# cambrian-mllm/cambrian

Hardware: NVIDIA H100
Metric: train_samples_per_sec (higher is better)
Workload: dtype bf16

## Files before the change

cambrian_b200/csrc/gemm.cu:

```cuda
#include "common.cuh"
#include <algorithm>
#include <cstring>
#include <cudaTypedefs.h>
#include <mutex>

namespace cb {

constexpr int BM = 128;
constexpr int BK = 64;
constexpr int GEMM_THREADS = 288;
constexpr int GROUP_M = 16;

struct GemmEpilogue {
  void* C;
  long long ldc, bsc;
  const bf16* bias;
  const bf16* colscale;
  const bf16* residual;
  long long ldr, bsr;
  float alpha;
  int out_fp32;
  int accumulate;
  int pair_ok;
  int tma_store;
};
constexpr int ACT_SWIGLU_PAIR = 5;

constexpr int STG_BYTES = 64 * 64 * 2;
constexpr int STAGING_BYTES = 2 * 2 * STG_BYTES;

template <int BN>
struct GemmCfg {
  static constexpr int A_BYTES = BM * BK * 2;
  static constexpr int B_BYTES = BN * BK * 2;
  static constexpr int STAGE_BYTES = A_BYTES + B_BYTES;
  static constexpr int STAGES = (BN == 256) ? 4 : (BN == 128 ? 6 : 8);
  static constexpr int SMEM_BYTES = STAGES * STAGE_BYTES + STAGING_BYTES + 1024  + 256 ;
  static_assert(SMEM_BYTES <= 232448, "exceeds the 227 KB of shared memory a CTA may use");
};

template <int ACT>
__device__ __forceinline__ float apply_act(float v) {
  if constexpr (ACT == 1) return gelu_erf(v);
  else if constexpr (ACT == 2) return gelu_tanh_fast(v);
  else if constexpr (ACT == 3) return quick_gelu(v);
  else if constexpr (ACT == 4) return silu(v);
  else return v;
}

__device__ __forceinline__ void tile_to_mn(int r, int m_blocks, int n_blocks, int& mb, int& nb) {
  const int tpg = GROUP_M * n_blocks;
  const int g = r / tpg;
  const int first = g * GROUP_M;
  const int gs = min(GROUP_M, m_blocks - first);
  const int w = r - g * tpg;
  mb = first + w % gs;
  nb = w / gs;
}

template <int BN, int ACT>
__device__ __forceinline__ void fuse_row(const GemmEpilogue& ep, long long c_off, long long r_off, int col0, int N,
                                         float* acc, int h) {
  constexpr int J = BN / 8;
#pragma unroll
  for (int j = 0; j < J; ++j) {
    acc[4 * j + 2 * h] *= ep.alpha;
    acc[4 * j + 2 * h + 1] *= ep.alpha;
  }
  if (ep.bias) {
#pragma unroll
    for (int j = 0; j < J; ++j) {
      const int col = col0 + 8 * j;
      if (col < N) {
        const float2 t = __bfloat1622float2(*reinterpret_cast<const __nv_bfloat162*>(ep.bias + col));
        acc[4 * j + 2 * h] += t.x;
        acc[4 * j + 2 * h + 1] += t.y;
      }
    }
  }
  if constexpr (ACT != 0) {
#pragma unroll
    for (int j = 0; j < J; ++j) {
      acc[4 * j + 2 * h] = apply_act<ACT>(acc[4 * j + 2 * h]);
      acc[4 * j + 2 * h + 1] = apply_act<ACT>(acc[4 * j + 2 * h + 1]);
    }
  }
  if (ep.colscale) {
#pragma unroll
    for (int j = 0; j < J; ++j) {
      const int col = col0 + 8 * j;
      if (col < N) {
        const float2 t = __bfloat1622float2(*reinterpret_cast<const __nv_bfloat162*>(ep.colscale + col));
        acc[4 * j + 2 * h] *= t.x;
        acc[4 * j + 2 * h + 1] *= t.y;
      }
    }
  }
  if (ep.residual) {
#pragma unroll
    for (int j = 0; j < J; ++j) {
      const int col = col0 + 8 * j;
      if (col < N) {
        const float2 t = __bfloat1622float2(*reinterpret_cast<const __nv_bfloat162*>(ep.residual + r_off + col));
        acc[4 * j + 2 * h] += t.x;
        acc[4 * j + 2 * h + 1] += t.y;
      }
    }
  }
  if (ep.accumulate && ep.out_fp32) {
    const float* cr = reinterpret_cast<const float*>(ep.C) + c_off;
#pragma unroll
    for (int j = 0; j < J; ++j) {
      const int col = col0 + 8 * j;
      if (col < N) {
        const float2 o = *reinterpret_cast<const float2*>(cr + col);
        acc[4 * j + 2 * h] += o.x;
        acc[4 * j + 2 * h + 1] += o.y;
      }
    }
  } else if (ep.accumulate) {
    const bf16* cr = reinterpret_cast<const bf16*>(ep.C) + c_off;
#pragma unroll
    for (int j = 0; j < J; ++j) {
      const int col = col0 + 8 * j;
      if (col < N) {
        const float2 o = __bfloat1622float2(*reinterpret_cast<const __nv_bfloat162*>(cr + col));
        acc[4 * j + 2 * h] += o.x;
        acc[4 * j + 2 * h + 1] += o.y;
      }
    }
  }
}

template <int BN>
__device__ __forceinline__ void store_row(const GemmEpilogue& ep, long long c_off, int col0, int N, const float* acc,
                                          int h) {
#pragma unroll
  for (int j = 0; j < BN / 8; ++j) {
    const int col = col0 + 8 * j;
    if (col >= N) continue;
    const float x = acc[4 * j + 2 * h], y = acc[4 * j + 2 * h + 1];
    if (ep.out_fp32) *reinterpret_cast<float2*>(reinterpret_cast<float*>(ep.C) + c_off + col) = make_float2(x, y);
    else *reinterpret_cast<__nv_bfloat162*>(reinterpret_cast<bf16*>(ep.C) + c_off + col) = __floats2bfloat162_rn(x, y);
  }
}

template <int ACT>
__device__ __forceinline__ void epilogue_elems(const GemmEpilogue& ep, long long c_off, long long r_off, int col, int N,
                                               float v0, float v1) {
  v0 *= ep.alpha;
  v1 *= ep.alpha;
#pragma unroll
  for (int e = 0; e < 2; ++e) {
    const int c = col + e;
    if (c >= N) break;
    float v = e ? v1 : v0;
    if (ep.bias) v += __bfloat162float(ep.bias[c]);
    v = apply_act<ACT>(v);
    if (ep.colscale) v *= __bfloat162float(ep.colscale[c]);
    if (ep.residual) v += __bfloat162float(ep.residual[r_off + c]);
    if (ep.out_fp32) {
      float* cp = reinterpret_cast<float*>(ep.C) + c_off + c;
      *cp = ep.accumulate ? *cp + v : v;
    } else {
      bf16* cp = reinterpret_cast<bf16*>(ep.C) + c_off + c;
      *cp = __float2bfloat16(ep.accumulate ? __bfloat162float(*cp) + v : v);
    }
  }
}

template <int BN, bool A_MN, bool B_MN, int ACT>
__global__ void __launch_bounds__(GEMM_THREADS, 1)
gemm_bf16_wgmma(const __grid_constant__ CUtensorMap tmA, const __grid_constant__ CUtensorMap tmB,
                const __grid_constant__ CUtensorMap tmC, const __grid_constant__ CUtensorMap tmAux, int M, int N, int K,
                int tiles, GemmEpilogue ep) {
  using Cfg = GemmCfg<BN>;
  constexpr int STAGES = Cfg::STAGES;
  constexpr bool SWIGLU = ACT == ACT_SWIGLU_PAIR;
  extern __shared__ uint8_t smem_raw[];
  const uint32_t smem_base = (smem_u32(smem_raw) + 1023u) & ~1023u;
  const uint32_t stg_base = smem_base + STAGES * Cfg::STAGE_BYTES;
  const uint32_t bar_base = stg_base + STAGING_BYTES;
  auto full_bar = [&](int s) { return bar_base + 8u * s; };
  auto empty_bar = [&](int s) { return bar_base + 8u * (STAGES + s); };

  const int warp = threadIdx.x >> 5;
  const int lane = threadIdx.x & 31;
  const int m_blocks = (M + BM - 1) / BM;
  const int n_blocks = SWIGLU ? (N / 2) / (BN / 2) : (N + BN - 1) / BN;
  const int tiles_per_batch = m_blocks * n_blocks;
  const int num_kb = (K + BK - 1) / BK;

  if (warp == 8 && lane == 0) {
    tma_prefetch_desc(&tmA);
    tma_prefetch_desc(&tmB);
    for (int s = 0; s < STAGES; ++s) {
      mbar_init(full_bar(s), 1);
      mbar_init(empty_bar(s), 2);
    }
    mbar_fence_init();
  }
  __syncthreads();

  if (warp == 8) {
    if (lane == 0) {
      int stage = 0;
      uint32_t phase = 0;
      for (int r = blockIdx.x; r < tiles; r += gridDim.x) {
        const int b = r / tiles_per_batch;
        int mb, nb;
        tile_to_mn(r - b * tiles_per_batch, m_blocks, n_blocks, mb, nb);
        const int m0 = mb * BM;
        for (int kb = 0; kb < num_kb; ++kb) {
          mbar_wait(empty_bar(stage), phase ^ 1u);
          const uint32_t sa = smem_base + stage * Cfg::STAGE_BYTES;
          const uint32_t sb = sa + Cfg::A_BYTES;
          mbar_arrive_expect_tx(full_bar(stage), Cfg::STAGE_BYTES);
          const int k0 = kb * BK;
          if (!A_MN) {
            tma_load_3d(sa, &tmA, full_bar(stage), k0, m0, b);
          } else {
#pragma unroll
            for (int i = 0; i < BM / 64; ++i)
              tma_load_3d(sa + i * (64 * BK * 2), &tmA, full_bar(stage), m0 + 64 * i, k0, b);
          }
          if (SWIGLU) {
            tma_load_3d(sb, &tmB, full_bar(stage), k0, nb * (BN / 2), 0);
            tma_load_3d(sb + (BN / 2) * BK * 2, &tmB, full_bar(stage), k0, N / 2 + nb * (BN / 2), 0);
          } else if (!B_MN) {
            tma_load_3d(sb, &tmB, full_bar(stage), k0, nb * BN, b);
          } else {
#pragma unroll
            for (int i = 0; i < BN / 64; ++i)
              tma_load_3d(sb + i * (64 * BK * 2), &tmB, full_bar(stage), nb * BN + 64 * i, k0, b);
          }
          if (++stage == STAGES) {
            stage = 0;
            phase ^= 1u;
          }
        }
      }
    }
    return;
  }

  const int wg = warp >> 2;
  const bool wg_leader = (threadIdx.x & 127) == 0;
  const int srow = (warp & 3) * 16 + (lane >> 2);
  const int cq = 2 * (lane & 3);
  const uint32_t stg = stg_base + wg * (2 * STG_BYTES);
  uint32_t q = 0;
  if (wg_leader && ep.tma_store) {
    tma_prefetch_desc(&tmC);
    if (SWIGLU) tma_prefetch_desc(&tmAux);
  }

  auto store_subtile = [&](const CUtensorMap* map, int x, int x_end, int y, int z, auto pair) {
    const uint32_t buf = stg + (q & 1u) * STG_BYTES;
#pragma unroll
    for (int h = 0; h < 2; ++h) {
      const int row = srow + 8 * h;
#pragma unroll
      for (int j = 0; j < 8; ++j) {
        const __nv_bfloat162 v = pair(j, h);
        st_shared_b32(buf + row * 128 + ((j ^ (row & 7)) << 4) + 2 * cq, *reinterpret_cast<const uint32_t*>(&v));
      }
    }
    fence_proxy_async_smem();
    if (wg_leader) bulk_wait_read<0>();
    named_bar_sync(1 + wg, 128);
    if (wg_leader && x < x_end && y < M) {
      tma_store_3d(map, buf, x, y, z);
      bulk_commit();
    }
    ++q;
  };

  float acc[BN / 2];
  int stage = 0;
  uint32_t phase = 0;
  for (int r = blockIdx.x; r < tiles; r += gridDim.x) {
    const int b = r / tiles_per_batch;
    int mb, nb;
    tile_to_mn(r - b * tiles_per_batch, m_blocks, n_blocks, mb, nb);
    const int m0 = mb * BM;
#pragma unroll
    for (int i = 0; i < BN / 2; ++i) acc[i] = 0.f;
    int prev_stage = -1;
    for (int kb = 0; kb < num_kb; ++kb) {
      mbar_wait(full_bar(stage), phase);
      const uint32_t sa = smem_base + stage * Cfg::STAGE_BYTES + wg * (64 * 128);
      const uint32_t sb = smem_base + stage * Cfg::STAGE_BYTES + Cfg::A_BYTES;
      reg_fence(acc);
      wgmma_fence();
#pragma unroll
      for (int k = 0; k < BK / 16; ++k) {
        const uint64_t adesc = A_MN ? make_smem_desc_sw128(sa + k * 2048, 64 * BK * 2, 1024)
                                    : make_smem_desc_sw128(sa + k * 32, 0, 1024);
        const uint64_t bdesc = B_MN ? make_smem_desc_sw128(sb + k * 2048, 64 * BK * 2, 1024)
                                    : make_smem_desc_sw128(sb + k * 32, 0, 1024);
        WgmmaSS<BN, A_MN ? 1 : 0, B_MN ? 1 : 0>::mma(acc, adesc, bdesc, 1u);
      }
      wgmma_commit();
      wgmma_wait<1>();
      reg_fence(acc);
      if (prev_stage >= 0 && wg_leader) mbar_arrive(empty_bar(prev_stage));
      prev_stage = stage;
      if (++stage == STAGES) {
        stage = 0;
        phase ^= 1u;
      }
    }
    wgmma_wait<0>();
    reg_fence(acc);
    if (wg_leader) mbar_arrive(empty_bar(prev_stage));

    const int y0 = m0 + wg * 64;
    if constexpr (SWIGLU) {
      constexpr int JH = BN / 16;
      const int F = N >> 1;
      const int f0 = nb * (BN / 2);
#pragma unroll
      for (int s = 0; s < BN / 128; ++s)
        store_subtile(&tmC, f0 + 64 * s, N, y0, 0, [&](int j, int h) {
          return __floats2bfloat162_rn(acc[4 * (8 * s + j) + 2 * h], acc[4 * (8 * s + j) + 2 * h + 1]);
        });
#pragma unroll
      for (int s = 0; s < BN / 128; ++s)
        store_subtile(&tmC, F + f0 + 64 * s, N, y0, 0, [&](int j, int h) {
          return __floats2bfloat162_rn(acc[4 * (JH + 8 * s + j) + 2 * h], acc[4 * (JH + 8 * s + j) + 2 * h + 1]);
        });
#pragma unroll
      for (int s = 0; s < BN / 128; ++s)
        store_subtile(&tmAux, f0 + 64 * s, F, y0, 0, [&](int j, int h) {
          const float2 g = __bfloat1622float2(
              __floats2bfloat162_rn(acc[4 * (8 * s + j) + 2 * h], acc[4 * (8 * s + j) + 2 * h + 1]));
          const float2 u = __bfloat1622float2(
              __floats2bfloat162_rn(acc[4 * (JH + 8 * s + j) + 2 * h], acc[4 * (JH + 8 * s + j) + 2 * h + 1]));
          return __floats2bfloat162_rn(silu(g.x) * u.x, silu(g.y) * u.y);
        });
    } else {
      const int n0 = nb * BN;
#pragma unroll
      for (int h = 0; h < 2; ++h) {
        const int row = y0 + srow + 8 * h;
        if (row >= M) continue;
        const long long c_off = static_cast<long long>(b) * ep.bsc + static_cast<long long>(row) * ep.ldc;
        const long long r_off = static_cast<long long>(b) * ep.bsr + static_cast<long long>(row) * ep.ldr;
        if (ep.pair_ok) {
          fuse_row<BN, ACT>(ep, c_off, r_off, n0 + cq, N, acc, h);
          if (!ep.tma_store) store_row<BN>(ep, c_off, n0 + cq, N, acc, h);
          continue;
        }
#pragma unroll
        for (int j = 0; j < BN / 8; ++j) {
          if (n0 + 8 * j >= N) break;
          epilogue_elems<ACT>(ep, c_off, r_off, n0 + 8 * j + cq, N, acc[4 * j + 2 * h], acc[4 * j + 2 * h + 1]);
        }
      }
      if (ep.tma_store) {
#pragma unroll
        for (int s = 0; s < BN / 64; ++s)
          store_subtile(&tmC, n0 + 64 * s, N, y0, b, [&](int j, int h) {
            return __floats2bfloat162_rn(acc[4 * (8 * s + j) + 2 * h], acc[4 * (8 * s + j) + 2 * h + 1]);
          });
      }
    }
  }
  if (wg_leader) bulk_wait<0>();
}

static PFN_cuTensorMapEncodeTiled_v12000 get_encode_fn() {
  static PFN_cuTensorMapEncodeTiled_v12000 fn = nullptr;
  static std::once_flag once;
  std::call_once(once, [] {
    void* p = nullptr;
    cudaDriverEntryPointQueryResult q;
    if (cudaGetDriverEntryPoint("cuTensorMapEncodeTiled", &p, cudaEnableDefault, &q) == cudaSuccess &&
        q == cudaDriverEntryPointSuccess)
      fn = reinterpret_cast<PFN_cuTensorMapEncodeTiled_v12000>(p);
  });
  return fn;
}

int make_tmap_bf16_3d(CUtensorMap* out, const void* base, uint64_t inner, uint64_t rows, uint64_t batch,
                      uint64_t ld_elems, uint64_t batch_stride_elems, uint32_t box_rows) {
  auto fn = get_encode_fn();
  if (!fn) return set_error(CB_ERR_CUDA, "cuTensorMapEncodeTiled entry point not available");
  if ((reinterpret_cast<uintptr_t>(base) & 15u) != 0)
    return set_error(CB_ERR_INVALID, "TMA operand base must be 16-byte aligned");
  if ((ld_elems % 8) != 0 || (batch > 1 && (batch_stride_elems % 8) != 0))
    return set_error(CB_ERR_INVALID, "TMA operand strides must be multiples of 8 elements (ld=%llu)",
                     (unsigned long long)ld_elems);
  cuuint64_t dims[3] = {inner, rows, batch};
  cuuint64_t bs = (batch > 1) ? batch_stride_elems * 2 : ld_elems * 2 * (rows ? rows : 1);
  cuuint64_t strides[2] = {ld_elems * 2, bs};
  cuuint32_t box[3] = {64, box_rows, 1};
  cuuint32_t estr[3] = {1, 1, 1};
  CUresult r = fn(out, CU_TENSOR_MAP_DATA_TYPE_BFLOAT16, 3, const_cast<void*>(base), dims, strides, box,
                  estr, CU_TENSOR_MAP_INTERLEAVE_NONE, CU_TENSOR_MAP_SWIZZLE_128B,
                  CU_TENSOR_MAP_L2_PROMOTION_L2_256B, CU_TENSOR_MAP_FLOAT_OOB_FILL_NONE);
  if (r == CUDA_ERROR_INVALID_CONTEXT) {
    cudaFree(0);
    r = fn(out, CU_TENSOR_MAP_DATA_TYPE_BFLOAT16, 3, const_cast<void*>(base), dims, strides, box, estr,
           CU_TENSOR_MAP_INTERLEAVE_NONE, CU_TENSOR_MAP_SWIZZLE_128B, CU_TENSOR_MAP_L2_PROMOTION_L2_256B,
           CU_TENSOR_MAP_FLOAT_OOB_FILL_NONE);
  }
  if (r != CUDA_SUCCESS) return set_error(CB_ERR_CUDA, "cuTensorMapEncodeTiled failed (%d)", (int)r);
  return CB_OK;
}

struct GemmMaps {
  CUtensorMap a, b, c, aux;
};

template <int BN, bool A_MN, bool B_MN, int ACT>
static int launch_gemm(const GemmMaps& tm, int M, int N, int K, int batch, const GemmEpilogue& ep,
                       cudaStream_t stream) {
  using Cfg = GemmCfg<BN>;
  auto kern = gemm_bf16_wgmma<BN, A_MN, B_MN, ACT>;
  static bool attr_set = false;
  if (!attr_set) {
    cudaError_t e = cudaFuncSetAttribute(kern, cudaFuncAttributeMaxDynamicSharedMemorySize, Cfg::SMEM_BYTES);
    if (e != cudaSuccess) return set_error(CB_ERR_CUDA, "gemm smem attr: %s", cudaGetErrorString(e));
    attr_set = true;
  }
  const int n_blocks = (ACT == ACT_SWIGLU_PAIR) ? (N / 2) / (BN / 2) : (N + BN - 1) / BN;
  const long long tiles = (long long)((M + BM - 1) / BM) * n_blocks * batch;
  CB_CHECK_ARG(tiles < (1LL << 31), "gemm: %lld tiles exceed the grid", tiles);
  const unsigned grid = (unsigned)std::min<long long>(tiles, device_sm_count());
  kern<<<grid, GEMM_THREADS, Cfg::SMEM_BYTES, stream>>>(tm.a, tm.b, tm.c, tm.aux, M, N, K, (int)tiles, ep);
  CB_CUDA_LAUNCH_CHECK("gemm_bf16_wgmma");
  return CB_OK;
}

template <int BN>
static int dispatch_major(int a_mn, int b_mn, int act, const GemmMaps& tm, int M, int N, int K, int batch,
                          const GemmEpilogue& ep, cudaStream_t stream) {
  if (!a_mn && !b_mn) {
    switch (act) {
      case 1: return launch_gemm<BN, false, false, 1>(tm, M, N, K, batch, ep, stream);
      case 2: return launch_gemm<BN, false, false, 2>(tm, M, N, K, batch, ep, stream);
      case 3: return launch_gemm<BN, false, false, 3>(tm, M, N, K, batch, ep, stream);
      case 4: return launch_gemm<BN, false, false, 4>(tm, M, N, K, batch, ep, stream);
      default: return launch_gemm<BN, false, false, 0>(tm, M, N, K, batch, ep, stream);
    }
  }
  if (!a_mn && b_mn) return launch_gemm<BN, false, true, 0>(tm, M, N, K, batch, ep, stream);
  if (a_mn && !b_mn) return launch_gemm<BN, true, false, 0>(tm, M, N, K, batch, ep, stream);
  return launch_gemm<BN, true, true, 0>(tm, M, N, K, batch, ep, stream);
}

int gemm_bf16(const void* A, const void* B, void* C, int M, int N, int K, int batch, long long lda,
              long long ldb, long long ldc, long long bsa, long long bsb, long long bsc, int a_mn, int b_mn,
              const void* bias, const void* colscale, const void* residual, long long ldr, long long bsr,
              float alpha, int act, int out_fp32, int accumulate, int force_bn, cudaStream_t stream) {
  CB_CHECK_ARG(M > 0 && N > 0 && K > 0 && batch > 0, "gemm: empty problem M=%d N=%d K=%d batch=%d", M, N, K,
               batch);
  CB_CHECK_ARG(A && B && C, "gemm: null operand");
  CB_CHECK_ARG(act >= 0 && act <= 4, "gemm: unknown activation %d", act);
  CB_CHECK_ARG(act == 0 || (!a_mn && !b_mn), "gemm: a fused activation needs K-major operands (forward layout)");
  CB_CHECK_ARG(force_bn == 0 || force_bn == 64 || force_bn == 128 || force_bn == 256, "gemm: bad BLOCK_N %d", force_bn);
  int bn = force_bn;
  if (bn == 0) {
    const int sms = device_sm_count();
    const long long mb = (M + BM - 1) / BM;
    auto tiles = [&](int b_n) { return mb * ((N + b_n - 1) / b_n) * batch; };
    if (N > 128 && tiles(256) >= (long long)(sms * 7) / 10) bn = 256;
    else if (N > 64 && tiles(128) >= (long long)(sms * 6) / 10) bn = 128;
    else if (N > 128 && tiles(64) > 2LL * sms) bn = 128;
    else bn = 64;
  }
  GemmMaps tm;
  std::memset(&tm, 0, sizeof(tm));
  int rc;
  if (!a_mn) rc = make_tmap_bf16_3d(&tm.a, A, K, M, batch, lda, bsa, BM);
  else       rc = make_tmap_bf16_3d(&tm.a, A, M, K, batch, lda, bsa, BK);
  if (rc) return rc;
  if (!b_mn) rc = make_tmap_bf16_3d(&tm.b, B, K, N, batch, ldb, bsb, bn);
  else       rc = make_tmap_bf16_3d(&tm.b, B, N, K, batch, ldb, bsb, BK);
  if (rc) return rc;
  GemmEpilogue ep;
  ep.C = C; ep.ldc = ldc; ep.bsc = bsc;
  ep.bias = static_cast<const bf16*>(bias);
  ep.colscale = static_cast<const bf16*>(colscale);
  ep.residual = static_cast<const bf16*>(residual);
  ep.ldr = ldr; ep.bsr = bsr;
  ep.alpha = alpha; ep.out_fp32 = out_fp32; ep.accumulate = accumulate;
  const unsigned calign = out_fp32 ? 7u : 3u;
  bool pair = (N % 2 == 0) && (ldc % 2 == 0) && (bsc % 2 == 0) && ((reinterpret_cast<uintptr_t>(C) & calign) == 0);
  if (residual)
    pair = pair && (ldr % 2 == 0) && (bsr % 2 == 0) && ((reinterpret_cast<uintptr_t>(residual) & 3u) == 0);
  if (bias) pair = pair && ((reinterpret_cast<uintptr_t>(bias) & 3u) == 0);
  if (colscale) pair = pair && ((reinterpret_cast<uintptr_t>(colscale) & 3u) == 0);
  ep.pair_ok = pair ? 1 : 0;
  const bool tma = pair && !out_fp32 && ((reinterpret_cast<uintptr_t>(C) & 15u) == 0) && ldc % 8 == 0 &&
                   (batch == 1 || (bsc > 0 && bsc % 8 == 0));
  if (tma && (rc = make_tmap_bf16_3d(&tm.c, C, N, M, batch, ldc, bsc, 64))) return rc;
  ep.tma_store = tma ? 1 : 0;
  switch (bn) {
    case 256: return dispatch_major<256>(a_mn, b_mn, act, tm, M, N, K, batch, ep, stream);
    case 128: return dispatch_major<128>(a_mn, b_mn, act, tm, M, N, K, batch, ep, stream);
    default:  return dispatch_major<64>(a_mn, b_mn, act, tm, M, N, K, batch, ep, stream);
  }
}

int gemm_swiglu_bf16(const void* A, const void* W, void* gu_out, void* act_out, int M, int F, int K, long long lda,
                     long long ldw, long long ld_gu, long long ld_act, cudaStream_t stream) {
  CB_CHECK_ARG(M > 0 && F > 0 && K > 0, "gemm_swiglu: empty problem M=%d F=%d K=%d", M, F, K);
  CB_CHECK_ARG(A && W && gu_out && act_out, "gemm_swiglu: null operand");
  CB_CHECK_ARG(F % 128 == 0, "gemm_swiglu: F=%d must be a multiple of 128 (whole 128-feature tiles, 16-byte aligned halves)", F);
  CB_CHECK_ARG(ld_gu % 8 == 0 && ld_act % 8 == 0 && ((reinterpret_cast<uintptr_t>(gu_out) & 15u) == 0) &&
                   ((reinterpret_cast<uintptr_t>(act_out) & 15u) == 0),
               "gemm_swiglu: outputs must be 16-byte aligned with ld %% 8 == 0");
  const int N = 2 * F;
  constexpr int BN = 256;
  GemmMaps tm;
  int rc;
  if ((rc = make_tmap_bf16_3d(&tm.a, A, K, M, 1, lda, 0, BM))) return rc;
  if ((rc = make_tmap_bf16_3d(&tm.b, W, K, N, 1, ldw, 0, BN / 2))) return rc;
  if ((rc = make_tmap_bf16_3d(&tm.c, gu_out, N, M, 1, ld_gu, 0, 64))) return rc;
  if ((rc = make_tmap_bf16_3d(&tm.aux, act_out, F, M, 1, ld_act, 0, 64))) return rc;
  GemmEpilogue ep;
  ep.C = gu_out; ep.ldc = ld_gu; ep.bsc = 0;
  ep.bias = nullptr; ep.colscale = nullptr; ep.residual = nullptr; ep.ldr = 0; ep.bsr = 0;
  ep.alpha = 1.0f; ep.out_fp32 = 0; ep.accumulate = 0; ep.pair_ok = 1; ep.tma_store = 1;
  return launch_gemm<BN, false, false, ACT_SWIGLU_PAIR>(tm, M, N, K, 1, ep, stream);
}

}
```

Measured before the change: 7.951.

## Add ping-pong warpgroup GEMM for BN=128 and TMA-loaded residual/accumulate epilogue

Adds a 384-thread ping-pong kernel for BN=128 tiles. In it, two consumer warpgroups each own a full 128x128 tile and take turns on the mainloop through order barriers, so one group's epilogue overlaps the other's MMAs. Register budgets are rebalanced with setmaxnreg. The epilogue can now bring residual or existing output tiles into shared memory with TMA and add them before a TMA store, replacing per-thread global loads. The BN heuristic also moves some 256-wide cases to 128 when padding is large or for activation GEMMs with moderate K. The cost is more barrier complexity and higher register pressure.

New measurement: 7.979 (median of 6 runs). About the same (+0.3%).

```diff
diff --git a/cambrian_b200/csrc/gemm.cu b/cambrian_b200/csrc/gemm.cu
--- a/cambrian_b200/csrc/gemm.cu
+++ b/cambrian_b200/csrc/gemm.cu
@@ -9,6 +9,8 @@
 constexpr int BM = 128;
 constexpr int BK = 64;
 constexpr int GEMM_THREADS = 288;
+constexpr int PP_THREADS = 384;
+constexpr int PP_BN = 128;
 constexpr int GROUP_M = 16;
 
 struct GemmEpilogue {
@@ -23,6 +25,7 @@
   int accumulate;
   int pair_ok;
   int tma_store;
+  int tma_src;
 };
 constexpr int ACT_SWIGLU_PAIR = 5;
 
@@ -96,7 +99,7 @@
       }
     }
   }
-  if (ep.residual) {
+  if (ep.residual && ep.tma_src != 1) {
 #pragma unroll
     for (int j = 0; j < J; ++j) {
       const int col = col0 + 8 * j;
@@ -107,7 +110,8 @@
       }
     }
   }
-  if (ep.accumulate && ep.out_fp32) {
+  if (ep.tma_src == 2) {
+  } else if (ep.accumulate && ep.out_fp32) {
     const float* cr = reinterpret_cast<const float*>(ep.C) + c_off;
 #pragma unroll
     for (int j = 0; j < J; ++j) {
@@ -169,6 +173,216 @@
   }
 }
 
+template <int BN, bool A_MN, bool B_MN, bool SWIGLU>
+__device__ __forceinline__ void produce_tiles(const CUtensorMap* tmA, const CUtensorMap* tmB, uint32_t smem_base,
+                                              uint32_t bar_base, int N, int tiles, int m_blocks, int n_blocks,
+                                              int num_kb) {
+  using Cfg = GemmCfg<BN>;
+  constexpr int STAGES = Cfg::STAGES;
+  auto full_bar = [&](int s) { return bar_base + 8u * s; };
+  auto empty_bar = [&](int s) { return bar_base + 8u * (STAGES + s); };
+  const int tiles_per_batch = m_blocks * n_blocks;
+  int stage = 0;
+  uint32_t phase = 0;
+  for (int r = blockIdx.x; r < tiles; r += gridDim.x) {
+    const int b = r / tiles_per_batch;
+    int mb, nb;
+    tile_to_mn(r - b * tiles_per_batch, m_blocks, n_blocks, mb, nb);
+    const int m0 = mb * BM;
+    for (int kb = 0; kb < num_kb; ++kb) {
+      mbar_wait(empty_bar(stage), phase ^ 1u);
+      const uint32_t sa = smem_base + stage * Cfg::STAGE_BYTES;
+      const uint32_t sb = sa + Cfg::A_BYTES;
+      mbar_arrive_expect_tx(full_bar(stage), Cfg::STAGE_BYTES);
+      const int k0 = kb * BK;
+      if (!A_MN) {
+        tma_load_3d(sa, tmA, full_bar(stage), k0, m0, b);
+      } else {
+#pragma unroll
+        for (int i = 0; i < BM / 64; ++i)
+          tma_load_3d(sa + i * (64 * BK * 2), tmA, full_bar(stage), m0 + 64 * i, k0, b);
+      }
+      if (SWIGLU) {
+        tma_load_3d(sb, tmB, full_bar(stage), k0, nb * (BN / 2), 0);
+        tma_load_3d(sb + (BN / 2) * BK * 2, tmB, full_bar(stage), k0, N / 2 + nb * (BN / 2), 0);
+      } else if (!B_MN) {
+        tma_load_3d(sb, tmB, full_bar(stage), k0, nb * BN, b);
+      } else {
+#pragma unroll
+        for (int i = 0; i < BN / 64; ++i)
+          tma_load_3d(sb + i * (64 * BK * 2), tmB, full_bar(stage), nb * BN + 64 * i, k0, b);
+      }
+      if (++stage == STAGES) {
+        stage = 0;
+        phase ^= 1u;
+      }
+    }
+  }
+}
+
+template <int BN, bool A_MN, bool B_MN>
+__device__ __forceinline__ void mma_kblock(float* acc, uint32_t sa, uint32_t sb) {
+#pragma unroll
+  for (int k = 0; k < BK / 16; ++k) {
+    const uint64_t adesc = A_MN ? make_smem_desc_sw128(sa + k * 2048, 64 * BK * 2, 1024)
+                                : make_smem_desc_sw128(sa + k * 32, 0, 1024);
+    const uint64_t bdesc = B_MN ? make_smem_desc_sw128(sb + k * 2048, 64 * BK * 2, 1024)
+                                : make_smem_desc_sw128(sb + k * 32, 0, 1024);
+    WgmmaSS<BN, A_MN ? 1 : 0, B_MN ? 1 : 0>::mma(acc, adesc, bdesc, 1u);
+  }
+}
+
+struct SubtileStore {
+  uint32_t stg;
+  uint32_t q;
+  uint32_t ld_bar;
+  uint32_t ld_phase;
+  int srow;
+  int cq;
+  int wg, M;
+  bool leader;
+
+  static __device__ __forceinline__ SubtileStore make(uint32_t stg_base, uint32_t ld_bars, int wg, int M) {
+    const int warp = (threadIdx.x >> 5) & 3, lane = threadIdx.x & 31;
+    return SubtileStore{stg_base + wg * (2 * STG_BYTES), 0u, ld_bars + 16u * wg, 0u, warp * 16 + (lane >> 2),
+                        2 * (lane & 3), wg, M, (threadIdx.x & 127) == 0};
+  }
+
+  template <int BN>
+  __device__ __forceinline__ void add_and_store(const CUtensorMap* src, const CUtensorMap* dst, int n0, int N, int y,
+                                                int z, const float* acc) {
+    constexpr int S = BN / 64;
+    auto load = [&](int s) {
+      const uint32_t b = (q + s) & 1u;
+      const uint32_t bar = ld_bar + 8u * b;
+      if (n0 + 64 * s < N && y < M) {
+        mbar_arrive_expect_tx(bar, STG_BYTES);
+        tma_load_3d(stg + b * STG_BYTES, src, bar, n0 + 64 * s, y, z);
+      } else {
+        mbar_arrive(bar);
+      }
+    };
+    if (leader) {
+      bulk_wait_read<0>();
+      load(0);
+      if (S > 1) load(1);
+    }
+#pragma unroll
+    for (int s = 0; s < S; ++s) {
+      const uint32_t b = (q + s) & 1u;
+      const uint32_t buf = stg + b * STG_BYTES;
+      mbar_wait(ld_bar + 8u * b, (ld_phase >> b) & 1u);
+      ld_phase ^= 1u << b;
+#pragma unroll
+      for (int h = 0; h < 2; ++h) {
+        const int row = srow + 8 * h;
+#pragma unroll
+        for (int j = 0; j < 8; ++j) {
+          const uint32_t addr = buf + row * 128 + ((j ^ (row & 7)) << 4) + 2 * cq;
+          uint32_t raw;
+          asm volatile("ld.shared.b32 %0, [%1];" : "=r"(raw) : "r"(addr) : "memory");
+          const float2 o = __bfloat1622float2(*reinterpret_cast<const __nv_bfloat162*>(&raw));
+          const __nv_bfloat162 v =
+              __floats2bfloat162_rn(acc[4 * (8 * s + j) + 2 * h] + o.x, acc[4 * (8 * s + j) + 2 * h + 1] + o.y);
+          st_shared_b32(addr, *reinterpret_cast<const uint32_t*>(&v));
+        }
+      }
+      fence_proxy_async_smem();
+      named_bar_sync(1 + wg, 128);
+      if (leader) {
+        if (n0 + 64 * s < N && y < M) {
+          tma_store_3d(dst, buf, n0 + 64 * s, y, z);
+          bulk_commit();
+        }
+        if (s + 2 < S) {
+          bulk_wait_read<0>();
+          load(s + 2);
+        }
+      }
+    }
+    q += S;
+  }
+  template <typename Pair>
+  __device__ __forceinline__ void operator()(const CUtensorMap* map, int x, int x_end, int y, int z, Pair pair) {
+    const uint32_t buf = stg + (q & 1u) * STG_BYTES;
+#pragma unroll
+    for (int h = 0; h < 2; ++h) {
+      const int row = srow + 8 * h;
+#pragma unroll
+      for (int j = 0; j < 8; ++j) {
+        const __nv_bfloat162 v = pair(j, h);
+        st_shared_b32(buf + row * 128 + ((j ^ (row & 7)) << 4) + 2 * cq, *reinterpret_cast<const uint32_t*>(&v));
+      }
+    }
+    fence_proxy_async_smem();
+    if (leader) bulk_wait_read<0>();
+    named_bar_sync(1 + wg, 128);
+    if (leader && x < x_end && y < M) {
+      tma_store_3d(map, buf, x, y, z);
+      bulk_commit();
+    }
+    ++q;
+  }
+};
+
+template <int BN, int ACT>
+__device__ __forceinline__ void epilogue_64(const GemmEpilogue& ep, const CUtensorMap* tmC, const CUtensorMap* tmAux,
+                                            int M, int N, int b, int nb, int y0, float* acc, SubtileStore& st) {
+  constexpr bool SWIGLU = ACT == ACT_SWIGLU_PAIR;
+  if constexpr (SWIGLU) {
+    constexpr int JH = BN / 16;
+    const int F = N >> 1;
+    const int f0 = nb * (BN / 2);
+#pragma unroll
+    for (int s = 0; s < BN / 128; ++s)
+      st(tmC, f0 + 64 * s, N, y0, 0, [&](int j, int h) {
+        return __floats2bfloat162_rn(acc[4 * (8 * s + j) + 2 * h], acc[4 * (8 * s + j) + 2 * h + 1]);
+      });
+#pragma unroll
+    for (int s = 0; s < BN / 128; ++s)
+      st(tmC, F + f0 + 64 * s, N, y0, 0, [&](int j, int h) {
+        return __floats2bfloat162_rn(acc[4 * (JH + 8 * s + j) + 2 * h], acc[4 * (JH + 8 * s + j) + 2 * h + 1]);
+      });
+#pragma unroll
+    for (int s = 0; s < BN / 128; ++s)
+      st(tmAux, f0 + 64 * s, F, y0, 0, [&](int j, int h) {
+        const float2 g = __bfloat1622float2(
+            __floats2bfloat162_rn(acc[4 * (8 * s + j) + 2 * h], acc[4 * (8 * s + j) + 2 * h + 1]));
+        const float2 u = __bfloat1622float2(
+            __floats2bfloat162_rn(acc[4 * (JH + 8 * s + j) + 2 * h], acc[4 * (JH + 8 * s + j) + 2 * h + 1]));
+        return __floats2bfloat162_rn(silu(g.x) * u.x, silu(g.y) * u.y);
+      });
+  } else {
+    const int n0 = nb * BN;
+#pragma unroll
+    for (int h = 0; h < 2; ++h) {
+      const int row = y0 + st.srow + 8 * h;
+      if (row >= M) continue;
+      const long long c_off = static_cast<long long>(b) * ep.bsc + static_cast<long long>(row) * ep.ldc;
+      const long long r_off = static_cast<long long>(b) * ep.bsr + static_cast<long long>(row) * ep.ldr;
+      if (ep.pair_ok) {
+        fuse_row<BN, ACT>(ep, c_off, r_off, n0 + st.cq, N, acc, h);
+        if (!ep.tma_store) store_row<BN>(ep, c_off, n0 + st.cq, N, acc, h);
+        continue;
+      }
+#pragma unroll
+      for (int j = 0; j < BN / 8; ++j) {
+        if (n0 + 8 * j >= N) break;
+        epilogue_elems<ACT>(ep, c_off, r_off, n0 + 8 * j + st.cq, N, acc[4 * j + 2 * h], acc[4 * j + 2 * h + 1]);
+      }
+    }
+    if (ep.tma_src) {
+      st.add_and_store<BN>(ep.tma_src == 1 ? tmAux : tmC, tmC, n0, N, y0, b, acc);
+    } else if (ep.tma_store) {
+#pragma unroll
+      for (int s = 0; s < BN / 64; ++s)
+        st(tmC, n0 + 64 * s, N, y0, b, [&](int j, int h) {
+          return __floats2bfloat162_rn(acc[4 * (8 * s + j) + 2 * h], acc[4 * (8 * s + j) + 2 * h + 1]);
+        });
+    }
+  }
+}
+
 template <int BN, bool A_MN, bool B_MN, int ACT>
 __global__ void __launch_bounds__(GEMM_THREADS, 1)
 gemm_bf16_wgmma(const __grid_constant__ CUtensorMap tmA, const __grid_constant__ CUtensorMap tmB,
@@ -183,6 +397,8 @@
   const uint32_t bar_base = stg_base + STAGING_BYTES;
   auto full_bar = [&](int s) { return bar_base + 8u * s; };
   auto empty_bar = [&](int s) { return bar_base + 8u * (STAGES + s); };
+  const uint32_t ld_bars = bar_base + 8u * (2 * STAGES + 2);
+  static_assert(8 * (2 * STAGES + 6) <= 256, "barriers fit the barrier area");
 
   const int warp = threadIdx.x >> 5;
   const int lane = threadIdx.x & 31;
@@ -198,83 +414,24 @@
       mbar_init(full_bar(s), 1);
       mbar_init(empty_bar(s), 2);
     }
+    for (int i = 0; i < 4; ++i) mbar_init(ld_bars + 8u * i, 1);
     mbar_fence_init();
   }
   __syncthreads();
 
   if (warp == 8) {
-    if (lane == 0) {
-      int stage = 0;
-      uint32_t phase = 0;
-      for (int r = blockIdx.x; r < tiles; r += gridDim.x) {
-        const int b = r / tiles_per_batch;
-        int mb, nb;
-        tile_to_mn(r - b * tiles_per_batch, m_blocks, n_blocks, mb, nb);
-        const int m0 = mb * BM;
-        for (int kb = 0; kb < num_kb; ++kb) {
-          mbar_wait(empty_bar(stage), phase ^ 1u);
-          const uint32_t sa = smem_base + stage * Cfg::STAGE_BYTES;
-          const uint32_t sb = sa + Cfg::A_BYTES;
-          mbar_arrive_expect_tx(full_bar(stage), Cfg::STAGE_BYTES);
-          const int k0 = kb * BK;
-          if (!A_MN) {
-            tma_load_3d(sa, &tmA, full_bar(stage), k0, m0, b);
-          } else {
-#pragma unroll
-            for (int i = 0; i < BM / 64; ++i)
-              tma_load_3d(sa + i * (64 * BK * 2), &tmA, full_bar(stage), m0 + 64 * i, k0, b);
-          }
-          if (SWIGLU) {
-            tma_load_3d(sb, &tmB, full_bar(stage), k0, nb * (BN / 2), 0);
-            tma_load_3d(sb + (BN / 2) * BK * 2, &tmB, full_bar(stage), k0, N / 2 + nb * (BN / 2), 0);
-          } else if (!B_MN) {
-            tma_load_3d(sb, &tmB, full_bar(stage), k0, nb * BN, b);
-          } else {
-#pragma unroll
-            for (int i = 0; i < BN / 64; ++i)
-              tma_load_3d(sb + i * (64 * BK * 2), &tmB, full_bar(stage), nb * BN + 64 * i, k0, b);
-          }
-          if (++stage == STAGES) {
-            stage = 0;
-            phase ^= 1u;
-          }
-        }
-      }
-    }
+    if (lane == 0)
+      produce_tiles<BN, A_MN, B_MN, SWIGLU>(&tmA, &tmB, smem_base, bar_base, N, tiles, m_blocks, n_blocks, num_kb);
     return;
   }
 
   const int wg = warp >> 2;
   const bool wg_leader = (threadIdx.x & 127) == 0;
-  const int srow = (warp & 3) * 16 + (lane >> 2);
-  const int cq = 2 * (lane & 3);
-  const uint32_t stg = stg_base + wg * (2 * STG_BYTES);
-  uint32_t q = 0;
   if (wg_leader && ep.tma_store) {
     tma_prefetch_desc(&tmC);
     if (SWIGLU) tma_prefetch_desc(&tmAux);
   }
-
-  auto store_subtile = [&](const CUtensorMap* map, int x, int x_end, int y, int z, auto pair) {
-    const uint32_t buf = stg + (q & 1u) * STG_BYTES;
-#pragma unroll
-    for (int h = 0; h < 2; ++h) {
-      const int row = srow + 8 * h;
-#pragma unroll
-      for (int j = 0; j < 8; ++j) {
-        const __nv_bfloat162 v = pair(j, h);
-        st_shared_b32(buf + row * 128 + ((j ^ (row & 7)) << 4) + 2 * cq, *reinterpret_cast<const uint32_t*>(&v));
-      }
-    }
-    fence_proxy_async_smem();
-    if (wg_leader) bulk_wait_read<0>();
-    named_bar_sync(1 + wg, 128);
-    if (wg_leader && x < x_end && y < M) {
-      tma_store_3d(map, buf, x, y, z);
-      bulk_commit();
-    }
-    ++q;
-  };
+  SubtileStore st = SubtileStore::make(stg_base, ld_bars, wg, M);
 
   float acc[BN / 2];
   int stage = 0;
@@ -283,24 +440,15 @@
     const int b = r / tiles_per_batch;
     int mb, nb;
     tile_to_mn(r - b * tiles_per_batch, m_blocks, n_blocks, mb, nb);
-    const int m0 = mb * BM;
 #pragma unroll
     for (int i = 0; i < BN / 2; ++i) acc[i] = 0.f;
     int prev_stage = -1;
     for (int kb = 0; kb < num_kb; ++kb) {
       mbar_wait(full_bar(stage), phase);
-      const uint32_t sa = smem_base + stage * Cfg::STAGE_BYTES + wg * (64 * 128);
-      const uint32_t sb = smem_base + stage * Cfg::STAGE_BYTES + Cfg::A_BYTES;
+      const uint32_t sa = smem_base + stage * Cfg::STAGE_BYTES;
       reg_fence(acc);
       wgmma_fence();
-#pragma unroll
-      for (int k = 0; k < BK / 16; ++k) {
-        const uint64_t adesc = A_MN ? make_smem_desc_sw128(sa + k * 2048, 64 * BK * 2, 1024)
-                                    : make_smem_desc_sw128(sa + k * 32, 0, 1024);
-        const uint64_t bdesc = B_MN ? make_smem_desc_sw128(sb + k * 2048, 64 * BK * 2, 1024)
-                                    : make_smem_desc_sw128(sb + k * 32, 0, 1024);
-        WgmmaSS<BN, A_MN ? 1 : 0, B_MN ? 1 : 0>::mma(acc, adesc, bdesc, 1u);
-      }
+      mma_kblock<BN, A_MN, B_MN>(acc, sa + wg * (64 * 128), sa + Cfg::A_BYTES);
       wgmma_commit();
       wgmma_wait<1>();
       reg_fence(acc);
@@ -314,58 +462,107 @@
     wgmma_wait<0>();
     reg_fence(acc);
     if (wg_leader) mbar_arrive(empty_bar(prev_stage));
-
-    const int y0 = m0 + wg * 64;
-    if constexpr (SWIGLU) {
-      constexpr int JH = BN / 16;
-      const int F = N >> 1;
-      const int f0 = nb * (BN / 2);
-#pragma unroll
-      for (int s = 0; s < BN / 128; ++s)
-        store_subtile(&tmC, f0 + 64 * s, N, y0, 0, [&](int j, int h) {
-          return __floats2bfloat162_rn(acc[4 * (8 * s + j) + 2 * h], acc[4 * (8 * s + j) + 2 * h + 1]);
-        });
-#pragma unroll
-      for (int s = 0; s < BN / 128; ++s)
-        store_subtile(&tmC, F + f0 + 64 * s, N, y0, 0, [&](int j, int h) {
-          return __floats2bfloat162_rn(acc[4 * (JH + 8 * s + j) + 2 * h], acc[4 * (JH + 8 * s + j) + 2 * h + 1]);
-        });
-#pragma unroll
-      for (int s = 0; s < BN / 128; ++s)
-        store_subtile(&tmAux, f0 + 64 * s, F, y0, 0, [&](int j, int h) {
-          const float2 g = __bfloat1622float2(
-              __floats2bfloat162_rn(acc[4 * (8 * s + j) + 2 * h], acc[4 * (8 * s + j) + 2 * h + 1]));
-          const float2 u = __bfloat1622float2(
-              __floats2bfloat162_rn(acc[4 * (JH + 8 * s + j) + 2 * h], acc[4 * (JH + 8 * s + j) + 2 * h + 1]));
-          return __floats2bfloat162_rn(silu(g.x) * u.x, silu(g.y) * u.y);
-        });
-    } else {
-      const int n0 = nb * BN;
-#pragma unroll
-      for (int h = 0; h < 2; ++h) {
-        const int row = y0 + srow + 8 * h;
-        if (row >= M) continue;
-        const long long c_off = static_cast<long long>(b) * ep.bsc + static_cast<long long>(row) * ep.ldc;
-        const long long r_off = static_cast<long long>(b) * ep.bsr + static_cast<long long>(row) * ep.ldr;
-        if (ep.pair_ok) {
-          fuse_row<BN, ACT>(ep, c_off, r_off, n0 + cq, N, acc, h);
-          if (!ep.tma_store) store_row<BN>(ep, c_off, n0 + cq, N, acc, h);
-          continue;
-        }
-#pragma unroll
-        for (int j = 0; j < BN / 8; ++j) {
-          if (n0 + 8 * j >= N) break;
-          epilogue_elems<ACT>(ep, c_off, r_off, n0 + 8 * j + cq, N, acc[4 * j + 2 * h], acc[4 * j + 2 * h + 1]);
-        }
-      }
-      if (ep.tma_store) {
-#pragma unroll
-        for (int s = 0; s < BN / 64; ++s)
-          store_subtile(&tmC, n0 + 64 * s, N, y0, b, [&](int j, int h) {
-            return __floats2bfloat162_rn(acc[4 * (8 * s + j) + 2 * h], acc[4 * (8 * s + j) + 2 * h + 1]);
-          });
-      }
-    }
+    epilogue_64<BN, ACT>(ep, &tmC, &tmAux, M, N, b, nb, mb * BM + wg * 64, acc, st);
+  }
+  if (wg_leader) bulk_wait<0>();
+}
+
+template <bool A_MN, bool B_MN, int ACT>
+__global__ void __launch_bounds__(PP_THREADS, 1)
+gemm_bf16_pingpong(const __grid_constant__ CUtensorMap tmA, const __grid_constant__ CUtensorMap tmB,
+                   const __grid_constant__ CUtensorMap tmC, const __grid_constant__ CUtensorMap tmAux, int M, int N,
+                   int K, int tiles, GemmEpilogue ep) {
+  constexpr int BN = PP_BN;
+  using Cfg = GemmCfg<BN>;
+  constexpr int STAGES = Cfg::STAGES;
+  static_assert(8 * (2 * STAGES + 6) <= 256, "the ring's, the order and the staging-load barriers fit the barrier area");
+  constexpr bool SWIGLU = ACT == ACT_SWIGLU_PAIR;
+  extern __shared__ uint8_t smem_raw[];
+  const uint32_t smem_base = (smem_u32(smem_raw) + 1023u) & ~1023u;
+  const uint32_t stg_base = smem_base + STAGES * Cfg::STAGE_BYTES;
+  const uint32_t bar_base = stg_base + STAGING_BYTES;
+  auto full_bar = [&](int s) { return bar_base + 8u * s; };
+  auto empty_bar = [&](int s) { return bar_base + 8u * (STAGES + s); };
+  auto order_bar = [&](int w) { return bar_base + 8u * (2 * STAGES + w); };
+  const uint32_t ld_bars = bar_base + 8u * (2 * STAGES + 2);
+
+  const int warp = threadIdx.x >> 5;
+  const int lane = threadIdx.x & 31;
+  const int m_blocks = (M + BM - 1) / BM;
+  const int n_blocks = SWIGLU ? (N / 2) / (BN / 2) : (N + BN - 1) / BN;
+  const int tiles_per_batch = m_blocks * n_blocks;
+  const int num_kb = (K + BK - 1) / BK;
+
+  if (warp == 8 && lane == 0) {
+    tma_prefetch_desc(&tmA);
+    tma_prefetch_desc(&tmB);
+    for (int s = 0; s < STAGES; ++s) {
+      mbar_init(full_bar(s), 1);
+      mbar_init(empty_bar(s), 1);
+    }
+    mbar_init(order_bar(0), 1);
+    mbar_init(order_bar(1), 1);
+    for (int i = 0; i < 4; ++i) mbar_init(ld_bars + 8u * i, 1);
+    mbar_fence_init();
+  }
+  __syncthreads();
+
+  if (warp >= 8) {
+    setmaxnreg_dec<40>();
+    if (warp == 8 && lane == 0)
+      produce_tiles<BN, A_MN, B_MN, SWIGLU>(&tmA, &tmB, smem_base, bar_base, N, tiles, m_blocks, n_blocks, num_kb);
+    return;
+  }
+
+  setmaxnreg_inc<232>();
+  const int wg = warp >> 2;
+  const bool wg_leader = (threadIdx.x & 127) == 0;
+  if (wg_leader && ep.tma_store) {
+    tma_prefetch_desc(&tmC);
+    if (SWIGLU) tma_prefetch_desc(&tmAux);
+  }
+  SubtileStore st = SubtileStore::make(stg_base, ld_bars, wg, M);
+
+  float acc[BN];
+  uint32_t order_phase = 0;
+  for (int t = wg, r = blockIdx.x + wg * gridDim.x; r < tiles; t += 2, r += 2 * gridDim.x) {
+    const int b = r / tiles_per_batch;
+    int mb, nb;
+    tile_to_mn(r - b * tiles_per_batch, m_blocks, n_blocks, mb, nb);
+    const long long f0 = (long long)t * num_kb;
+    int stage = (int)(f0 % STAGES);
+    uint32_t phase = (uint32_t)((f0 / STAGES) & 1);
+#pragma unroll
+    for (int i = 0; i < BN; ++i) acc[i] = 0.f;
+    if (t > 0) {
+      mbar_wait(order_bar(wg), order_phase);
+      order_phase ^= 1u;
+    }
+    int prev_stage = -1;
+    for (int kb = 0; kb < num_kb; ++kb) {
+      mbar_wait(full_bar(stage), phase);
+      const uint32_t sa = smem_base + stage * Cfg::STAGE_BYTES;
+      reg_fence(acc);
+      wgmma_fence();
+      mma_kblock<BN, A_MN, B_MN>(acc, sa, sa + Cfg::A_BYTES);
+      mma_kblock<BN, A_MN, B_MN>(acc + BN / 2, sa + 64 * 128, sa + Cfg::A_BYTES);
+      wgmma_commit();
+      wgmma_wait<1>();
+      reg_fence(acc);
+      if (prev_stage >= 0 && wg_leader) mbar_arrive(empty_bar(prev_stage));
+      prev_stage = stage;
+      if (++stage == STAGES) {
+        stage = 0;
+        phase ^= 1u;
+      }
+    }
+    if (wg_leader) mbar_arrive(order_bar(wg ^ 1));
+    wgmma_wait<0>();
+    reg_fence(acc);
+    if (wg_leader) mbar_arrive(empty_bar(prev_stage));
+#pragma unroll
+    for (int i = 0; i < 2; ++i)
+      epilogue_64<BN, ACT>(ep, &tmC, &tmAux, M, N, b, nb, mb * BM + 64 * i, acc + i * (BN / 2), st);
   }
   if (wg_leader) bulk_wait<0>();
 }
@@ -418,10 +615,14 @@
 static int launch_gemm(const GemmMaps& tm, int M, int N, int K, int batch, const GemmEpilogue& ep,
                        cudaStream_t stream) {
   using Cfg = GemmCfg<BN>;
-  auto kern = gemm_bf16_wgmma<BN, A_MN, B_MN, ACT>;
+  constexpr bool PP = BN == PP_BN;
+  constexpr int SMEM = Cfg::SMEM_BYTES;
+  void (*kern)(CUtensorMap, CUtensorMap, CUtensorMap, CUtensorMap, int, int, int, int, GemmEpilogue);
+  if constexpr (PP) kern = gemm_bf16_pingpong<A_MN, B_MN, ACT>;
+  else kern = gemm_bf16_wgmma<BN, A_MN, B_MN, ACT>;
   static bool attr_set = false;
   if (!attr_set) {
-    cudaError_t e = cudaFuncSetAttribute(kern, cudaFuncAttributeMaxDynamicSharedMemorySize, Cfg::SMEM_BYTES);
+    cudaError_t e = cudaFuncSetAttribute(kern, cudaFuncAttributeMaxDynamicSharedMemorySize, SMEM);
     if (e != cudaSuccess) return set_error(CB_ERR_CUDA, "gemm smem attr: %s", cudaGetErrorString(e));
     attr_set = true;
   }
@@ -429,8 +630,8 @@
   const long long tiles = (long long)((M + BM - 1) / BM) * n_blocks * batch;
   CB_CHECK_ARG(tiles < (1LL << 31), "gemm: %lld tiles exceed the grid", tiles);
   const unsigned grid = (unsigned)std::min<long long>(tiles, device_sm_count());
-  kern<<<grid, GEMM_THREADS, Cfg::SMEM_BYTES, stream>>>(tm.a, tm.b, tm.c, tm.aux, M, N, K, (int)tiles, ep);
-  CB_CUDA_LAUNCH_CHECK("gemm_bf16_wgmma");
+  kern<<<grid, PP ? PP_THREADS : GEMM_THREADS, SMEM, stream>>>(tm.a, tm.b, tm.c, tm.aux, M, N, K, (int)tiles, ep);
+  CB_CUDA_LAUNCH_CHECK(PP ? "gemm_bf16_pingpong" : "gemm_bf16_wgmma");
   return CB_OK;
 }
 
@@ -470,6 +671,8 @@
     else if (N > 64 && tiles(128) >= (long long)(sms * 6) / 10) bn = 128;
     else if (N > 128 && tiles(64) > 2LL * sms) bn = 128;
     else bn = 64;
+    const int pad = (256 - N % 256) % 256;
+    if (bn == 256 && N % 128 == 0 && (5 * pad > N || (act != 0 && K > 512 && K <= 1536))) bn = 128;
   }
   GemmMaps tm;
   std::memset(&tm, 0, sizeof(tm));
@@ -498,6 +701,14 @@
                    (batch == 1 || (bsc > 0 && bsc % 8 == 0));
   if (tma && (rc = make_tmap_bf16_3d(&tm.c, C, N, M, batch, ldc, bsc, 64))) return rc;
   ep.tma_store = tma ? 1 : 0;
+  ep.tma_src = 0;
+  if (tma && residual && !accumulate && ((reinterpret_cast<uintptr_t>(residual) & 15u) == 0) && ldr % 8 == 0 &&
+      (batch == 1 || (bsr > 0 && bsr % 8 == 0))) {
+    if ((rc = make_tmap_bf16_3d(&tm.aux, residual, N, M, batch, ldr, bsr, 64))) return rc;
+    ep.tma_src = 1;
+  } else if (tma && accumulate && !residual) {
+    ep.tma_src = 2;
+  }
   switch (bn) {
     case 256: return dispatch_major<256>(a_mn, b_mn, act, tm, M, N, K, batch, ep, stream);
     case 128: return dispatch_major<128>(a_mn, b_mn, act, tm, M, N, K, batch, ep, stream);
@@ -524,7 +735,7 @@
   GemmEpilogue ep;
   ep.C = gu_out; ep.ldc = ld_gu; ep.bsc = 0;
   ep.bias = nullptr; ep.colscale = nullptr; ep.residual = nullptr; ep.ldr = 0; ep.bsr = 0;
-  ep.alpha = 1.0f; ep.out_fp32 = 0; ep.accumulate = 0; ep.pair_ok = 1; ep.tma_store = 1;
+  ep.alpha = 1.0f; ep.out_fp32 = 0; ep.accumulate = 0; ep.pair_ok = 1; ep.tma_store = 1; ep.tma_src = 0;
   return launch_gemm<BN, false, false, ACT_SWIGLU_PAIR>(tm, M, N, K, 1, ep, stream);
 }
 
```
